# WoojuLee24/OA-DG

Measured on AMD Instinct MI355X. Metric: images/sec training, Faster R-CNN R50-FPN + OA-DG, 1024x2048, higher is better.
Workload: dtype bf16

## Files before the change

oa-dg_amd/csrc/conv_mfma.hip:

```cpp
#include <algorithm>
#include <vector>
#include "common.h"
#include <type_traits>
#include <stdlib.h>
#include "oadg_hip.h"

namespace {

constexpr int BM = 128, BN = 128, BK = 64;

struct ConvArgs {
    const unsigned short* x;
    const unsigned short* w;
    const float* bias;
    const unsigned short* res;
    unsigned short* y;
    const unsigned short* zeros;
    const unsigned short* mask;
    const unsigned char* bits_in;
    unsigned char* bits_out;
    float* colsum;
    int N, H, W, C, K, R, S, Ho, Wo, stride, pad, dil, relu;
    long M;
    int scatter, OH, OW, osh, osw, oph, opw;
    int res_up, lh, lw;
};

__device__ __forceinline__ long out_row(const ConvArgs& a, long m) {
    if (!a.scatter) return m;
    if (a.M <= 0x7fffffffL) {
        const unsigned t = (unsigned)m / (unsigned)a.Wo, wo = (unsigned)m - t * (unsigned)a.Wo;
        const unsigned n = t / (unsigned)a.Ho, ho = t - n * (unsigned)a.Ho;
        return ((long)n * a.OH + (long)ho * a.osh + a.oph) * a.OW + (long)wo * a.osw + a.opw;
    }
    const long t = m / a.Wo;
    const int wo = (int)(m - t * a.Wo);
    const long n = t / a.Ho;
    const int ho = (int)(t - n * a.Ho);
    return (n * a.OH + (long)ho * a.osh + a.oph) * a.OW + (long)wo * a.osw + a.opw;
}

#define OADG_UNIFORM_BRANCH() asm volatile("" ::: "memory")
template <bool POST>
__device__ __forceinline__ bf16x8 finish_piece(const ConvArgs& a, bf16x8 v, const bf16x8 rv, const bf16x8 mv,
                                               float* csum, unsigned mbits = 0xffu, size_t off = 0) {
    if (POST) {
        float f[8];
#pragma unroll
        for (int e = 0; e < 8; ++e) f[e] = bf16_to_f32((unsigned short)v[e]);
        if (a.res) {
            OADG_UNIFORM_BRANCH();
#pragma unroll
            for (int e = 0; e < 8; ++e) f[e] += bf16_to_f32((unsigned short)rv[e]);
            if (a.relu) {
                OADG_UNIFORM_BRANCH();
#pragma unroll
                for (int e = 0; e < 8; ++e) f[e] = fmaxf(f[e], 0.f);
            }
        }
        if (a.mask) {
            OADG_UNIFORM_BRANCH();
#pragma unroll
            for (int e = 0; e < 8; ++e)
                if (!(bf16_to_f32((unsigned short)mv[e]) > 0.f)) f[e] = 0.f;
        }
        if (a.bits_in) {
            OADG_UNIFORM_BRANCH();
#pragma unroll
            for (int e = 0; e < 8; ++e)
                if (!((mbits >> e) & 1u)) f[e] = 0.f;
        }
#pragma unroll
        for (int e = 0; e < 8; ++e) v[e] = (short)f32_to_bf16(f[e]);
    }
    if (a.colsum) {
        OADG_UNIFORM_BRANCH();
#pragma unroll
        for (int e = 0; e < 8; ++e) csum[e] += bf16_to_f32((unsigned short)v[e]);
    }
    if (a.bits_out) {
        OADG_UNIFORM_BRANCH();
        unsigned b = 0;
#pragma unroll
        for (int e = 0; e < 8; ++e) b |= (bf16_to_f32((unsigned short)v[e]) > 0.f ? 1u : 0u) << e;
        a.bits_out[off >> 3] = (unsigned char)b;
    }
    return v;
}

typedef __attribute__((address_space(3))) void* lds_ptr_t;
typedef const __attribute__((address_space(1))) void* gbl_ptr_t;

__device__ __forceinline__ void glds16(const void* g, void* l) {
    __builtin_amdgcn_global_load_lds((gbl_ptr_t)g, (lds_ptr_t)l, 16, 0, 0);
}

template <int TBN, bool POST, int NST, bool PW = false>
__device__ __forceinline__ void conv_igemm_body(const ConvArgs& a, const long bid, unsigned char* smem) {
    constexpr int WN = TBN / 64, WM = 4 / WN, AF = BM / WM / 32, NBP = TBN * 8 / 256;
    constexpr int TSTAGE = (BM + TBN) * BK * 2;
    const int tid = threadIdx.x, lane = tid & 63, wave = tid >> 6;
    const int wm = wave / WN, wn = wave % WN;
    const int n_tiles = a.K / TBN;
    const long m_tiles = (a.M + BM - 1) / BM;
    long mt;
    int nt;
    {
        const long xcd = bid & 7, j = bid >> 3;
        const long per = (m_tiles + 7) >> 3;
        nt = (int)(j % n_tiles);
        mt = PW ? (j / n_tiles) * 8 + xcd : xcd * per + j / n_tiles;
        if (j / n_tiles >= per || mt >= m_tiles) return;
    }
    const long m0 = mt * BM;
    const int k0 = nt * TBN;

    const int cpc = a.C / BK;
    const int nchunks = a.R * a.S * cpc;
    const unsigned short* a_base[4];
    int a_hi0[4], a_wi0[4];
    int seg[4];
    const unsigned short* b_base[4];
#pragma unroll
    for (int i = 0; i < 4; ++i) {
        const int q = i * 256 + tid;
        const int row = q >> 3, slot = q & 7;
        seg[i] = slot ^ ((row >> 1) & 7);
        const long m = m0 + row;
        if (PW) {
            a_base[i] = m < a.M ? a.x + (size_t)m * a.C : nullptr;
            a_hi0[i] = a_wi0[i] = 0;
        } else if (m < a.M) {
            int wo, ho, n;
            if (a.M <= 0x7fffffffL) {
                const unsigned t = (unsigned)m / (unsigned)a.Wo;
                wo = (int)((unsigned)m - t * (unsigned)a.Wo);
                n = (int)(t / (unsigned)a.Ho);
                ho = (int)(t - (unsigned)n * (unsigned)a.Ho);
            } else {
                wo = (int)(m % a.Wo);
                const long t = m / a.Wo;
                ho = (int)(t % a.Ho);
                n = (int)(t / a.Ho);
            }
            a_hi0[i] = ho * a.stride - a.pad;
            a_wi0[i] = wo * a.stride - a.pad;
            a_base[i] = a.x + ((long)n * a.H * a.W + (long)a_hi0[i] * a.W + a_wi0[i]) * a.C + seg[i] * 8;
        } else {
            a_base[i] = nullptr;
            a_hi0[i] = -(1 << 28);
            a_wi0[i] = 0;
        }
        b_base[i] = a.w + (size_t)(k0 + (row < TBN ? row : 0)) * a.R * a.S * a.C + seg[i] * 8;
    }

    int st_r = 0, st_s = 0, st_rs = 0, st_c0 = 0;
    auto stage = [&](int kc, int buf) {
        unsigned char* sa = smem + buf * TSTAGE;
        unsigned char* sb = sa + BM * BK * 2;
        if (PW) {
            const int c0 = kc * BK;
#pragma unroll
            for (int i = 0; i < 4; ++i)
                glds16(a_base[i] ? a_base[i] + c0 + seg[i] * 8 : a.zeros, sa + i * 4096 + wave * 1024);
#pragma unroll
            for (int i = 0; i < NBP; ++i) glds16(b_base[i] + c0, sb + i * 4096 + wave * 1024);
            return;
        }
        const int dr = st_r * a.dil, ds = st_s * a.dil;
        const long aoff = ((long)dr * a.W + ds) * a.C + st_c0;
        const long boff = (long)st_rs * a.C + st_c0;
#pragma unroll
        for (int i = 0; i < 4; ++i) {
            const bool ok = (unsigned)(a_hi0[i] + dr) < (unsigned)a.H && (unsigned)(a_wi0[i] + ds) < (unsigned)a.W;
            glds16(ok ? a_base[i] + aoff : a.zeros, sa + i * 4096 + wave * 1024);
        }
#pragma unroll
        for (int i = 0; i < NBP; ++i) glds16(b_base[i] + boff, sb + i * 4096 + wave * 1024);
// ... 264 lines not shown
        for (int p = 0; p < NS - 1; ++p) stage(range + p * ranges, p);
        request(range, 0);

        auto body = [&](int i, auto set_c) {
            constexpr int set = decltype(set_c)::value;
            const long sub = range + i * ranges;
            OADG_VMCNT((NS - 2) * G + (NS - 1) * (R + S));
            asm volatile("s_barrier" ::: "memory");
            stage(sub + (NS - 1) * ranges, (i + NS - 1) % NS);
            request(sub + ranges, set ^ 1);
            const unsigned char* at = ring + (i % NS) * SUB_BYTES;
            f32x4 acc[RT][CT];
#pragma unroll
            for (int rt = 0; rt < RT; ++rt)
#pragma unroll
                for (int ct = 0; ct < CT; ++ct) acc[rt][ct] = f32x4{0.f, 0.f, 0.f, 0.f};
#pragma unroll
            for (int ks = 0; ks < KS; ++ks) {
                bf16x8 pf[CT];
#pragma unroll
                for (int ct = 0; ct < CT; ++ct)
                    pf[ct] = *reinterpret_cast<const bf16x8*>(at + bbase[ct] + (bsw[ct] ^ (ks * 64)));
#pragma unroll
                for (int rt = 0; rt < RT; ++rt)
#pragma unroll
                    for (int ct = 0; ct < CT; ++ct)
                        acc[rt][ct] = __builtin_amdgcn_mfma_f32_16x16x32_bf16(wf[rt][ks], pf[ct], acc[rt][ct], 0, 0, 0);
            }
#pragma unroll
            for (int rt = 0; rt < RT; ++rt) {
                const f32x4 bv = *reinterpret_cast<const f32x4*>(sbias + rt * 16 + fq * 4);
#pragma unroll
                for (int ct = 0; ct < CT; ++ct) {
                    bf16x4 o;
#pragma unroll
                    for (int r = 0; r < 4; ++r) {
                        float v = acc[rt][ct][r] + bv[r];
                        if (a.relu && !RES) v = fmaxf(v, 0.f);
                        o[r] = (short)f32_to_bf16(v);
                    }
                    *reinterpret_cast<bf16x4*>(stg + (ct * 16 + fr) * STG_STRIDE + (rt * 16 + fq * 4) * 2) = o;
                }
            }
            asm volatile("" ::: "memory");
            if (POST) {
                OADG_VMCNT(S + G + R);
#pragma unroll
                for (int jj = 0; jj < NP; ++jj) {
                    if (RES) asm volatile("" : "+v"(rv[set][jj]));
                    if (BIN) asm volatile("" : "+v"(mb[set][jj]));
                }
            }
#pragma unroll
            for (int jj = 0; jj < NP; ++jj) {
                const int px = ppx + PPP * jj;
                bf16x8 v = *reinterpret_cast<const bf16x8*>(stg + px * STG_STRIDE + psl * 16);
                const size_t off = (size_t)sub * sub_stride + jj * row8 + lane_off;
                v = finish_piece<POST>(a, v, RES ? rv[set][jj] : bf16x8{0, 0, 0, 0, 0, 0, 0, 0}, bf16x8{0, 0, 0, 0, 0, 0, 0, 0},
                                       csum, BIN ? mb[set][jj] : 0xffu, off);
                asm volatile("global_store_dwordx4 %0, %1, off" ::"v"(a.y + off), "v"(v) : "memory");
            }
        };
        OADG_VMCNT(0);
        for (int i = 0; i < n_it; i += 2) {
            body(i, std::integral_constant<int, 0>{});
            if (i + 1 < n_it) body(i + 1, std::integral_constant<int, 1>{});
        }
    }
    if (a.colsum) {
#pragma unroll
        for (int e = 0; e < 8; ++e) {
            float t = csum[e];
#pragma unroll
            for (int sh = LPP; sh < 64; sh <<= 1) t += __shfl_xor(t, sh, 64);
            csum[e] = t;
        }
        if (lane < LPP) {
#pragma unroll
            for (int e = 0; e < 8; ++e) a.colsum[(size_t)range * a.K + kcol + lane * 8 + e] = csum[e];
        }
    }
}

long pw_stream_ranges(long M, int C, int K, int R, int S, int stride, int pad) {
    if (R != 1 || S != 1 || stride != 1 || pad != 0 || (C != 64 && C != 128 && C != 256 && C != 512)) return 0;
    const int kwg = C >= 512 ? 128 : 256;
    if (K % kwg != 0) return 0;
    const int ncol = K / kwg, sp = C >= 256 ? 16 : 32;
    if (ncol > 64 || (64 % ncol) != 0 || M % sp != 0) return 0;
    const long ranges = 512 / ncol;
    return (M / sp) >= 8 * ranges ? ranges : 0;
}

template <int C>
int launch_pw_stream(const ConvArgs& a, hipStream_t st) {
    using Geo = PwGeo<C>;
    const int ncol = a.K / (4 * Geo::KPW);
    const bool res = a.res != nullptr, bin = a.bits_in != nullptr, bout = a.bits_out != nullptr;
#define OADG_PWS(RE, BI, BO)                                                                                       \
    do {                                                                                                           \
        static bool attr = false;                                                                                  \
        if (!attr) {                                                                                               \
            hipError_t e = hipFuncSetAttribute((const void*)conv_pw_stream_kernel<C, RE, BI, BO>,                  \
                                               hipFuncAttributeMaxDynamicSharedMemorySize, Geo::LDS);              \
            if (e != hipSuccess) return (int)e;                                                                    \
            attr = true;                                                                                           \
        }                                                                                                          \
        hipLaunchKernelGGL((conv_pw_stream_kernel<C, RE, BI, BO>), dim3(Geo::GRID), dim3(256), Geo::LDS, st, a, ncol); \
    } while (0)
    if (res && bin && !bout) OADG_PWS(true, true, false);
    else if (res && !bin && bout) OADG_PWS(true, false, true);
    else if (res && !bin && !bout) OADG_PWS(true, false, false);
    else if (!res && bin && !bout) OADG_PWS(false, true, false);
    else if (!res && !bin && bout) OADG_PWS(false, false, true);
    else if (!res && !bin && !bout) OADG_PWS(false, false, false);
    else return OADG_EARG;
#undef OADG_PWS
    return OADG_OK;
}

constexpr int TM = 256, TN = 256;
constexpr int HALF_BYTES = 128 * BK * 2;
constexpr int BUF_BYTES = 4 * HALF_BYTES;

typedef float f32x4v __attribute__((ext_vector_type(4)));

struct TapState {
    int t, r, s, rs, c0;
};

template <bool POST, int NW>
__global__ __launch_bounds__(512) void conv_igemm256_kernel(ConvArgs a) {
    constexpr int TNW = NW * 128;
    extern __shared__ __attribute__((aligned(16))) unsigned char smem[];
    const int tid = threadIdx.x, lane = tid & 63;
    const int wave = __builtin_amdgcn_readfirstlane(tid >> 6);
    const int wr = wave >> 2, wc = wave & 3;
    const int n_tiles = a.K / TNW;
    const long m_tiles = (a.M + TM - 1) / TM;
    const long bid = blockIdx.x;
    long mt;
    int nt;
    {
        const long xcd = bid & 7, j = bid >> 3;
        const long per = (m_tiles + 7) >> 3;
        nt = (int)(j % n_tiles);
        mt = xcd * per + j / n_tiles;
        if (j / n_tiles >= per || mt >= m_tiles) return;
    }
    const long m0 = mt * TM;
    const int k0 = nt * TNW;
    const int nk = a.R * a.S * (a.C / BK);

    const unsigned short* pb[4];
    int hi0[4], wi0[4];
    const unsigned short* wb[4];
#pragma unroll
    for (int h = 0; h < 2; ++h)
#pragma unroll
        for (int i = 0; i < 2; ++i) {
            const int q = i * 512 + tid;
            const int row = q >> 3, lslot = (q & 7) ^ ((row >> 1) & 7);
            const long m = m0 + h * 128 + row;
            if (m < a.M) {
                const unsigned mu = (unsigned)m;
                const unsigned tq = mu / (unsigned)a.Wo;
                const int wo = (int)(mu - tq * (unsigned)a.Wo);
                const int n = (int)(tq / (unsigned)a.Ho);
                const int ho = (int)(tq - (unsigned)n * (unsigned)a.Ho);
                pb[h * 2 + i] = a.x + (size_t)n * a.H * a.W * a.C + lslot * 8;
                hi0[h * 2 + i] = ho * a.stride - a.pad;
                wi0[h * 2 + i] = wo * a.stride - a.pad;
            } else {
                pb[h * 2 + i] = a.x;
                hi0[h * 2 + i] = -(1 << 28);
                wi0[h * 2 + i] = 0;
            }
            wb[h * 2 + i] = a.w + (size_t)(k0 + (h & (NW - 1)) * 128 + row) * a.R * a.S * a.C + lslot * 8;
        }

    auto advance = [&](TapState& st) {
        st.t++;
        st.rs++;
        if (++st.s == a.S) {
            st.s = 0;
            if (++st.r == a.R) { st.r = 0; st.rs = 0; st.c0 += BK; }
        }
    };
    auto stage_pix = [&](int h, const TapState& st, int buf) {
        unsigned char* dst = smem + buf * BUF_BYTES + h * HALF_BYTES + wave * 1024;
        const bool live = st.t < nk;
#pragma unroll
        for (int i = 0; i < 2; ++i) {
            const int hi = hi0[h * 2 + i] + st.r * a.dil, wi = wi0[h * 2 + i] + st.s * a.dil;
            const bool ok = live && (unsigned)hi < (unsigned)a.H && (unsigned)wi < (unsigned)a.W;
            const unsigned short* src = ok ? pb[h * 2 + i] + ((hi * a.W + wi) * a.C + st.c0) : a.zeros;
            glds16(src, dst + i * 8192);
        }
    };
    auto stage_wgt = [&](int h, const TapState& st, int buf) {
        unsigned char* dst = smem + buf * BUF_BYTES + (2 + h) * HALF_BYTES + wave * 1024;
        const bool live = st.t < nk;
#pragma unroll
        for (int i = 0; i < 2; ++i) {
            const unsigned short* src = live ? wb[h * 2 + i] + (st.rs * a.C + st.c0) : a.zeros;
            glds16(src, dst + i * 8192);
        }
    };

    const int fr = lane & 15, fq = lane >> 4;
    int poff[4][2], woff[2][2];
#pragma unroll
    for (int it = 0; it < 4; ++it)
#pragma unroll
        for (int ks = 0; ks < 2; ++ks) {
            const int row = wr * 64 + it * 16 + fr;
            poff[it][ks] = row * 128 + (((ks * 4 + fq) ^ ((row >> 1) & 7)) << 4);
        }
#pragma unroll
    for (int jt = 0; jt < 2; ++jt)
#pragma unroll
        for (int ks = 0; ks < 2; ++ks) {
            const int row = wc * 32 + jt * 16 + fr;
            woff[jt][ks] = row * 128 + (((ks * 4 + fq) ^ ((row >> 1) & 7)) << 4);
        }

    f32x4v acc[NW][2][2][4];
#pragma unroll
    for (int x0 = 0; x0 < NW; ++x0)
#pragma unroll
        for (int x1 = 0; x1 < 2; ++x1)
#pragma unroll
            for (int x2 = 0; x2 < 2; ++x2)
#pragma unroll
                for (int x3 = 0; x3 < 4; ++x3) acc[x0][x1][x2][x3] = f32x4v{0.f, 0.f, 0.f, 0.f};

    bf16x8 pf[4][2], wf[NW][2][2];
    auto read_pix = [&](int h, int buf) {
        const unsigned char* base = smem + buf * BUF_BYTES + h * HALF_BYTES;
#pragma unroll
        for (int it = 0; it < 4; ++it)
#pragma unroll
            for (int ks = 0; ks < 2; ++ks) pf[it][ks] = *reinterpret_cast<const bf16x8*>(base + poff[it][ks]);
    };
    auto read_wgt = [&](int h, int buf) {
        const unsigned char* base = smem + buf * BUF_BYTES + (2 + h) * HALF_BYTES;
#pragma unroll
        for (int jt = 0; jt < 2; ++jt)
#pragma unroll
            for (int ks = 0; ks < 2; ++ks) wf[h][jt][ks] = *reinterpret_cast<const bf16x8*>(base + woff[jt][ks]);
    };
#define OADG_MFMA32(W_FIRST, PH_)                                                                            \
    do {                                                                                                     \
        asm volatile("s_waitcnt lgkmcnt(0)" ::: "memory");                                                   \
        asm volatile("s_barrier" ::: "memory");                                                              \
        __builtin_amdgcn_sched_barrier(0);                                                                   \
        __builtin_amdgcn_s_setprio(1);                                                                       \
        _Pragma("unroll") for (int hh = 0; hh < NW; ++hh)                                                    \
            _Pragma("unroll") for (int ks = 0; ks < 2; ++ks)                                                 \
                _Pragma("unroll") for (int jt = 0; jt < 2; ++jt)                                             \
                    _Pragma("unroll") for (int it = 0; it < 4; ++it)                                         \
                        acc[(hh ^ W_FIRST) & (NW - 1)][jt][PH_][it] = __builtin_amdgcn_mfma_f32_16x16x32_bf16(   \
                            wf[(hh ^ W_FIRST) & (NW - 1)][jt][ks], pf[it][ks],                               \
                            acc[(hh ^ W_FIRST) & (NW - 1)][jt][PH_][it], 0, 0, 0);                           \
        __builtin_amdgcn_s_setprio(0);                                                                       \
        __builtin_amdgcn_sched_barrier(0);                                                                   \
        asm volatile("s_barrier" ::: "memory");                                                              \
    } while (0)

    TapState s1{0, 0, 0, 0, 0};
    stage_pix(0, s1, 0);
    stage_wgt(0, s1, 0);
    if (NW == 2) stage_wgt(1, s1, 0);
    stage_pix(1, s1, 0);
    advance(s1);
    stage_pix(0, s1, 1);
    stage_wgt(0, s1, 1);
    TapState s2 = s1;
    advance(s2);
    asm volatile("s_waitcnt vmcnt(4)" ::: "memory");
    asm volatile("s_barrier" ::: "memory");
    if (wr == 1) asm volatile("s_barrier" ::: "memory");

    for (int t = 0; t < nk; ++t) {
        const int buf = t & 1;
        read_wgt(0, buf);
        if (NW == 2) read_wgt(1, buf);
        read_pix(0, buf);
        if (NW == 2) stage_wgt(1, s1, buf ^ 1);
        stage_pix(1, s1, buf ^ 1);
        OADG_MFMA32(0, 0);
        read_pix(1, buf);
        stage_pix(0, s2, buf);
        stage_wgt(0, s2, buf);
        asm volatile("s_waitcnt vmcnt(4)" ::: "memory");
        OADG_MFMA32(1, 1);
        s1 = s2;
        advance(s2);
    }
#undef OADG_MFMA32
    if (wr == 0) asm volatile("s_barrier" ::: "memory");
    asm volatile("s_waitcnt vmcnt(0)" ::: "memory");
    asm volatile("s_barrier" ::: "memory");

    {
        const int cq = lane >> 4;
#pragma unroll
        for (int wh = 0; wh < NW; ++wh)
#pragma unroll
            for (int jt = 0; jt < 2; ++jt) {
                const int ch = wh * 128 + wc * 32 + jt * 16 + 4 * cq;
                float bv[4] = {0.f, 0.f, 0.f, 0.f};
                if (a.bias) {
#pragma unroll
                    for (int e = 0; e < 4; ++e) bv[e] = a.bias[k0 + ch + e];
                }
#pragma unroll
                for (int ph = 0; ph < 2; ++ph)
#pragma unroll
                    for (int it = 0; it < 4; ++it) {
                        const int p = ph * 128 + wr * 64 + it * 16 + fr;
                        unsigned short o[4];
#pragma unroll
                        for (int e = 0; e < 4; ++e) {
                            float v = acc[wh][jt][ph][it][e] + bv[e];
                            if (a.relu && !a.res) v = fmaxf(v, 0.f);
                            o[e] = f32_to_bf16(v);
                        }
                        uint2 pk;
                        pk.x = (unsigned)o[0] | ((unsigned)o[1] << 16);
                        pk.y = (unsigned)o[2] | ((unsigned)o[3] << 16);
                        *reinterpret_cast<uint2*>(smem + p * (TNW * 2) + ((((ch >> 3) ^ (p & 15))) << 4) + ((ch >> 2) & 1) * 8) = pk;
                    }
            }
    }
    constexpr int NPIECE = (TM * TNW / 8) / 512, SL = TNW / 8;
    bf16x8 rv[POST ? NPIECE : 1], mv[POST ? NPIECE : 1];
    unsigned mb[POST ? NPIECE : 1];
    if (POST) {
#pragma unroll
        for (int it = 0; it < NPIECE; ++it) {
            const int q = it * 512 + tid;
            const long m = m0 + q / SL;
            const size_t off = (size_t)m * a.K + k0 + (q % SL) * 8;
            rv[it] = (a.res && m < a.M) ? *reinterpret_cast<const bf16x8*>(a.res + off) : bf16x8{0, 0, 0, 0, 0, 0, 0, 0};
            mv[it] = (a.mask && m < a.M) ? *reinterpret_cast<const bf16x8*>(a.mask + off) : bf16x8{0, 0, 0, 0, 0, 0, 0, 0};
            mb[it] = (a.bits_in && m < a.M) ? a.bits_in[off >> 3] : 0xffu;
        }
    } else {
        rv[0] = mv[0] = bf16x8{0, 0, 0, 0, 0, 0, 0, 0};
        mb[0] = 0xffu;
    }
    __syncthreads();
    float csum[8] = {0.f, 0.f, 0.f, 0.f, 0.f, 0.f, 0.f, 0.f};
#pragma unroll
    for (int it = 0; it < NPIECE; ++it) {
        const int q = it * 512 + tid;
        const int p = q / SL, sg = q % SL;
        const long m = m0 + p;
        if (m >= a.M) continue;
        bf16x8 v = *reinterpret_cast<const bf16x8*>(smem + p * (TNW * 2) + ((sg ^ (p & 15)) << 4));
        const size_t off = (size_t)m * a.K + k0 + sg * 8;
        *reinterpret_cast<bf16x8*>(a.y + off) = finish_piece<POST>(a, v, rv[POST ? it : 0], mv[POST ? it : 0], csum,
                                                                   mb[POST ? it : 0], off);
    }
    if (a.colsum) {
        float* red = reinterpret_cast<float*>(smem + 2 * BUF_BYTES);
#pragma unroll
        for (int e = 0; e < 8; ++e) red[(tid / SL) * TNW + (tid % SL) * 8 + e] = csum[e];
        __syncthreads();
        if (tid < TNW) {
            float t = 0.f;
#pragma unroll
            for (int g = 0; g < 512 / SL; ++g) t += red[g * TNW + tid];
            a.colsum[(size_t)mt * a.K + k0 + tid] = t;
        }
    }
}

}

namespace {
int auto_variant(long M, int H, int W, int C, int K, int nchunks, int R = 0, int S = 0, int stride = 0, int pad = 0) {
    constexpr bool narrow256 = false;
    const int tnw = K % TN == 0 ? TN : 128;
    const long big = ((M + TM - 1) / TM) * (K / tnw);
    const bool ok256 = (K % TN == 0 || (K == 128 && narrow256)) && big >= 256 && (long)H * W * C < (1L << 31) && M < (1L << 31);
    if (ok256 && nchunks >= 12) return 2;
    if (pw_stream_ranges(M, C, K, R, S, stride, pad) > 0) return 4;
    if (ok256 && nchunks >= 8) return 2;
    const long blocks128 = ((M + BM - 1) / BM) * ((K + 127) / 128);
    if (K % 128 == 0 && blocks128 <= 512 && nchunks >= 32) return 1;
    return 3;
}

static inline bool mask_bits_unused(const void* bits_in, const void* bits_out) { return bits_in != nullptr || bits_out != nullptr; }

int conv_launch(const void* x, const void* w, const float* bias, const void* residual, void* y, const void* zeros16,
                int N, int H, int W, int C, int K, int R, int S, int stride, int pad, int dil, int relu, int variant,
                void* stream, const void* mask = nullptr, float* colsum_part = nullptr, const int* sc = nullptr,
                const void* bits_in = nullptr, void* bits_out = nullptr) {
    if (!x || !w || !y || !zeros16) return OADG_EARG;
    if (N < 1 || H < 1 || W < 1 || R < 1 || S < 1 || stride < 1 || dil < 1 || pad < 0) return OADG_EARG;
    if (C % BK != 0 || K % 64 != 0) return OADG_EARG;
    if (variant < 0 || variant > 4 || (variant == 2 && K % 128 != 0)) return OADG_EARG;
    ConvArgs a;
    a.x = (const unsigned short*)x; a.w = (const unsigned short*)w; a.bias = bias;
    a.res = (const unsigned short*)residual; a.y = (unsigned short*)y; a.zeros = (const unsigned short*)zeros16;
    a.mask = (const unsigned short*)mask; a.colsum = colsum_part;
    a.bits_in = (const unsigned char*)bits_in; a.bits_out = (unsigned char*)bits_out;
    if ((bits_in || bits_out) && K % 8 != 0) return OADG_EARG;
    a.N = N; a.H = H; a.W = W; a.C = C; a.K = K; a.R = R; a.S = S; a.stride = stride; a.pad = pad; a.dil = dil;
    a.relu = relu & 1;
    a.Ho = (H + 2 * pad - dil * (R - 1) - 1) / stride + 1;
    a.Wo = (W + 2 * pad - dil * (S - 1) - 1) / stride + 1;
    a.scatter = 0; a.OH = a.Ho; a.OW = a.Wo; a.osh = a.osw = 1; a.oph = a.opw = 0;
    a.res_up = 0; a.lh = a.lw = 0;
    if (relu & 2) {
        auto lg = [](int v) { int l = 0; while ((1 << l) < v) ++l; return (1 << l) == v ? l : -1; };
        a.lh = lg(H); a.lw = lg(W);
        if (!residual || (H & 1) || (W & 1) || H < 2 || W < 2 || (long)N * H * W >= (1L << 31) || R != 1 || S != 1 || stride != 1 ||
            pad != 0 || sc || mask || mask_bits_unused(bits_in, bits_out))
            return OADG_EARG;
        a.res_up = (a.lh >= 1 && a.lw >= 1) ? 1 : 2;
        a.relu = relu & 1;
        if (variant == 0) variant = 4;
        if (variant != 4) return OADG_EARG;
    }
    if (sc) {
        if (stride != 1 || sc[0] < 1 || sc[1] < 1 || sc[4] < 1 || sc[5] < 1 || sc[6] < 0 || sc[7] < 0) return OADG_EARG;
        if ((long)(sc[0] - 1) * sc[4] + sc[6] >= sc[2] || (long)(sc[1] - 1) * sc[5] + sc[7] >= sc[3]) return OADG_EARG;
        a.Ho = sc[0]; a.Wo = sc[1];
        a.scatter = 1; a.OH = sc[2]; a.OW = sc[3]; a.osh = sc[4]; a.osw = sc[5]; a.oph = sc[6]; a.opw = sc[7];
        if (variant == 0 || variant == 2) variant = 3;
    }
    if (a.Ho < 1 || a.Wo < 1) return OADG_EARG;
    a.M = (long)N * a.Ho * a.Wo;
    const bool post = residual != nullptr || mask != nullptr || bits_in != nullptr;
    if (variant == 0) {
        variant = auto_variant(a.M, H, W, C, K, R * S * (C / BK), R, S, stride, pad);
        if (variant == 4 && (sc || mask || (bits_in && bits_out))) variant = 3;
    }
    if (variant == 2 && ((long)H * W * C >= (1L << 31) || a.M >= (1L << 31))) variant = 1;
    if (variant == 4) {
        if (sc || mask || (bits_in && bits_out) || pw_stream_ranges(a.M, C, K, R, S, stride, pad) == 0) return OADG_EARG;
        int rc = OADG_EARG;
        if (C == 64) rc = launch_pw_stream<64>(a, (hipStream_t)stream);
        else if (C == 128) rc = launch_pw_stream<128>(a, (hipStream_t)stream);
        else if (C == 256) rc = launch_pw_stream<256>(a, (hipStream_t)stream);
        else if (C == 512) rc = launch_pw_stream<512>(a, (hipStream_t)stream);
        if (rc != OADG_OK) return rc;
        OADG_LAUNCH_CHECK();
        return OADG_OK;
    }
    if (variant == 2) {
        static bool attr_set = false;
        if (!attr_set) {
            const void* fns[4] = {(const void*)conv_igemm256_kernel<false, 2>, (const void*)conv_igemm256_kernel<true, 2>,
                                  (const void*)conv_igemm256_kernel<false, 1>, (const void*)conv_igemm256_kernel<true, 1>};
            for (const void* f : fns) {
                hipError_t e = hipFuncSetAttribute(f, hipFuncAttributeMaxDynamicSharedMemorySize, 2 * BUF_BYTES + 16384);
                if (e != hipSuccess) return (int)e;
            }
            attr_set = true;
        }
        const int nw = K % TN == 0 ? 2 : 1;
        const long m_tiles = (a.M + TM - 1) / TM;
        const long blocks = ((m_tiles + 7) / 8) * 8 * (K / (nw * 128));
        if (blocks > 0x7fffffffL) return OADG_EARG;
#define OADG_L256(PO, NW_) \
    hipLaunchKernelGGL((conv_igemm256_kernel<PO, NW_>), dim3((unsigned)blocks), dim3(512), 2 * BUF_BYTES + 16384, (hipStream_t)stream, a)
        if (nw == 2) { if (post) OADG_L256(true, 2); else OADG_L256(false, 2); }
        else { if (post) OADG_L256(true, 1); else OADG_L256(false, 1); }
#undef OADG_L256
    } else {
        const long m_tiles = (a.M + BM - 1) / BM;
        constexpr long tbn64_max = 256;
        const int tbn = (K % BN == 0 && m_tiles * (K / BN) > tbn64_max) ? BN : 64;
        const long blocks = ((m_tiles + 7) / 8) * 8 * (K / tbn);
        if (blocks > 0x7fffffffL) return OADG_EARG;
        const bool one = variant == 3;
        const unsigned lds2 = 2 * (BM + tbn) * BK * 2, lds1 = (BM + tbn) * BK * 2 + 8192;
        hipStream_t st = (hipStream_t)stream;
#define OADG_L128(TB, PO, NS, LDS) \
    hipLaunchKernelGGL((conv_igemm_kernel<TB, PO, NS>), dim3((unsigned)blocks), dim3(256), LDS, st, a)
#define OADG_L128PW(TB, PO, LDS) \
    hipLaunchKernelGGL((conv_igemm_kernel<TB, PO, 1, true>), dim3((unsigned)blocks), dim3(256), LDS, st, a)
        const bool pw = one && R == 1 && S == 1 && stride == 1 && pad == 0 && !a.scatter;
        if (pw) {
            if (tbn == BN) { if (post) OADG_L128PW(128, true, lds1); else OADG_L128PW(128, false, lds1); }
            else { if (post) OADG_L128PW(64, true, lds1); else OADG_L128PW(64, false, lds1); }
        } else if (tbn == BN) {
            if (one) { if (post) OADG_L128(128, true, 1, lds1); else OADG_L128(128, false, 1, lds1); }
            else { if (post) OADG_L128(128, true, 2, lds2); else OADG_L128(128, false, 2, lds2); }
        } else {
            if (one) { if (post) OADG_L128(64, true, 1, lds1); else OADG_L128(64, false, 1, lds1); }
            else { if (post) OADG_L128(64, true, 2, lds2); else OADG_L128(64, false, 2, lds2); }
        }
#undef OADG_L128
#undef OADG_L128PW
    }
    OADG_LAUNCH_CHECK();
    return OADG_OK;
}
}

extern "C" int oadg_conv2d_nhwc_bf16(const void* x, const void* w, const float* bias, const void* residual,
                                     void* y, const void* zeros16, int N, int H, int W, int C, int K, int R,
                                     int S, int stride, int pad, int dil, int relu, void* stream) {
    return conv_launch(x, w, bias, residual, y, zeros16, N, H, W, C, K, R, S, stride, pad, dil, relu, 0, stream);
}

extern "C" int oadg_conv2d_auto_variant(int N, int H, int W, int C, int K, int R, int S, int stride, int pad, int dil) {
    if (N < 1 || H < 1 || W < 1 || R < 1 || S < 1 || stride < 1 || dil < 1 || pad < 0) return 0;
    if (C % BK != 0 || K % 64 != 0) return 0;
    const int Ho = (H + 2 * pad - dil * (R - 1) - 1) / stride + 1, Wo = (W + 2 * pad - dil * (S - 1) - 1) / stride + 1;
    if (Ho < 1 || Wo < 1) return 0;
    return auto_variant((long)N * Ho * Wo, H, W, C, K, R * S * (C / BK), R, S, stride, pad);
}

extern "C" int oadg_conv2d_nhwc_bf16_ex(const void* x, const void* w, const float* bias, const void* residual,
                                        void* y, const void* zeros16, int N, int H, int W, int C, int K, int R, int S,
                                        int stride, int pad, int dil, int relu, int variant, const void* mask,
                                        float* colsum_part, const void* mask_bits, void* relu_bits_out, void* stream) {
    return conv_launch(x, w, bias, residual, y, zeros16, N, H, W, C, K, R, S, stride, pad, dil, relu, variant, stream,
                       mask, colsum_part, nullptr, mask_bits, relu_bits_out);
}

extern "C" int oadg_conv2d_nhwc_bf16_scatter(const void* x, const void* w, const float* bias, const void* residual,
                                             void* y, const void* zeros16, int N, int H, int W, int C, int K, int R,
                                             int S, int pad, int dil, int relu, int out_h, int out_w, int OH, int OW,
                                             int osh, int osw, int oph, int opw, const void* mask,
                                             float* colsum_part, const void* mask_bits, void* stream) {
    const int sc[8] = {out_h, out_w, OH, OW, osh, osw, oph, opw};
    return conv_launch(x, w, bias, residual, y, zeros16, N, H, W, C, K, R, S, 1, pad, dil, relu, 3, stream, mask,
                       colsum_part, sc, mask_bits, nullptr);
}

extern "C" int oadg_conv2d_dgrad_s2_nhwc_bf16(const void* dy, const void* wt, const void* residual, void* dx,
                                              const void* zeros16, int N, int Ho, int Wo, int K, int C, int R, int H, int W,
                                              const void* mask, float* colsum_part, const void* mask_bits, void* stream) {
    if (!dy || !wt || !dx || !zeros16 || N < 1 || Ho < 1 || Wo < 1 || H < 1 || W < 1 || (R != 3 && R != 1)) return OADG_EARG;
    if (K % BK != 0 || C % 64 != 0 || (mask_bits && C % 8 != 0)) return OADG_EARG;
    static const int cls_tab[4][5] = {{0, 0, 1, 1, 0}, {0, 1, 1, 2, 1}, {1, 0, 2, 1, 3}, {1, 1, 2, 2, 5}};
    S2Args g;
    ConvArgs& a = g.base;
    a.x = (const unsigned short*)dy; a.w = nullptr; a.bias = nullptr; a.res = (const unsigned short*)residual;
    a.y = (unsigned short*)dx; a.zeros = (const unsigned short*)zeros16; a.mask = (const unsigned short*)mask;
    a.bits_in = (const unsigned char*)mask_bits; a.bits_out = nullptr; a.colsum = nullptr;
    a.N = N; a.H = Ho; a.W = Wo; a.C = K; a.K = C; a.R = 1; a.S = 1; a.stride = 1; a.pad = 0; a.dil = 1; a.relu = 0;
    a.Ho = a.Wo = 1; a.M = 0;
    a.scatter = 1; a.OH = H; a.OW = W; a.osh = 2; a.osw = 2; a.oph = a.opw = 0;
    a.res_up = 0; a.lh = a.lw = 0;
    const int tbn = (C % BN == 0) ? BN : 64;
    g.n_cls = 0;
    long blocks = 0, rows = 0;
    bool equal = true;
    long first_blocks = -1;
    for (int k = 0; k < (R == 3 ? 4 : 1); ++k) {
        const int ph = cls_tab[k][0], pw = cls_tab[k][1];
        const int ha = (H - ph + 1) / 2, wa = (W - pw + 1) / 2;
        if (ha < 1 || wa < 1) continue;
        if ((long)(ha - 1) * 2 + ph >= H || (long)(wa - 1) * 2 + pw >= W) return OADG_EARG;
        S2Class& c = g.cls[g.n_cls++];
        c.w = (const unsigned short*)wt + (size_t)cls_tab[k][4] * C * K;
        c.R = cls_tab[k][2]; c.S = cls_tab[k][3]; c.Ho = ha; c.Wo = wa; c.oph = ph; c.opw = pw;
        c.M = (long)N * ha * wa;
        const long m_tiles = (c.M + BM - 1) / BM;
        c.colsum = colsum_part ? colsum_part + (size_t)rows * C : nullptr;
        rows += m_tiles;
        const long b = ((m_tiles + 7) / 8) * 8 * (C / tbn);
        if (first_blocks < 0) first_blocks = b;
        equal = equal && b == first_blocks;
        if (blocks + b > 0x7fffffffL) return OADG_EARG;
        c.block0 = (int)blocks;
        blocks += b;
    }
    if (g.n_cls == 0) return OADG_OK;
    for (int k = g.n_cls; k < 4; ++k) g.cls[k] = g.cls[0];
    g.interleave = (g.n_cls == 4 && equal) ? 1 : 0;
    const bool post = residual != nullptr || mask != nullptr || mask_bits != nullptr;
    const unsigned lds1 = (BM + tbn) * BK * 2 + 8192;
    hipStream_t st = (hipStream_t)stream;
#define OADG_LS2(TB, PO) hipLaunchKernelGGL((conv_igemm_s2_kernel<TB, PO>), dim3((unsigned)blocks), dim3(256), lds1, st, g)
    if (tbn == BN) { if (post) OADG_LS2(128, true); else OADG_LS2(128, false); }
    else { if (post) OADG_LS2(64, true); else OADG_LS2(64, false); }
#undef OADG_LS2
    OADG_LAUNCH_CHECK();
    return OADG_OK;
}

extern "C" long oadg_conv2d_pixel_tiles(int N, int H, int W, int C, int K, int R, int S, int stride, int pad, int dil,
                                        int variant) {
    if (variant == 0) variant = oadg_conv2d_auto_variant(N, H, W, C, K, R, S, stride, pad, dil);
    if (variant == 0) return 0;
    const int Ho = (H + 2 * pad - dil * (R - 1) - 1) / stride + 1, Wo = (W + 2 * pad - dil * (S - 1) - 1) / stride + 1;
    const long M = (long)N * Ho * Wo;
    if (variant == 4) return pw_stream_ranges(M, C, K, R, S, stride, pad);
    return variant == 2 ? (M + TM - 1) / TM : (M + BM - 1) / BM;
}

extern "C" int oadg_conv2d_nhwc_bf16_variant(const void* x, const void* w, const float* bias, const void* residual,
                                             void* y, const void* zeros16, int N, int H, int W, int C, int K, int R,
                                             int S, int stride, int pad, int dil, int relu, int variant,
                                             void* stream) {
    return conv_launch(x, w, bias, residual, y, zeros16, N, H, W, C, K, R, S, stride, pad, dil, relu, variant, stream);
}

namespace {

struct WgradArgs {
    const unsigned short* x;
    const unsigned short* dy;
    float* part;
    const unsigned short* zeros;
    int N, H, W, C, K, R, S, Ho, Wo, stride, pad, dil, splits, chunks_per_split;
    int strip_rows;
    long P;
};
// ... 1148 lines not shown
```

Before: 144.4.

## Add row-segment staging path for 3x3 stride-1 convs in 256-tile igemm

Adds a specialized path in the 256-row implicit-GEMM conv kernel for 3x3, stride-1, pad-1 convolutions. It stages whole output-row segments plus a one-pixel halo into LDS once per kernel row and reuses them across the three horizontal taps by shifting fragment addresses. This replaces reloading pixels from global memory for every tap. It uses buffer loads with out-of-bounds offsets to zero-fill padding and is enabled by default when shape conditions hold, with an environment variable to disable it. The tradeoff is more complex LDS addressing and a narrower set of shapes where it applies.

New measurement: 146.2, median of 6. No clear change (+1.2%).

```diff
diff --git a/oa-dg_amd/csrc/conv_mfma.hip b/oa-dg_amd/csrc/conv_mfma.hip
--- a/oa-dg_amd/csrc/conv_mfma.hip
+++ b/oa-dg_amd/csrc/conv_mfma.hip
@@ -24,6 +24,7 @@
     long M;
     int scatter, OH, OW, osh, osw, oph, opw;
     int res_up, lh, lw;
+    int rows;
 };
 
 __device__ __forceinline__ long out_row(const ConvArgs& a, long m) {
@@ -594,78 +595,7 @@
     const int k0 = nt * TNW;
     const int nk = a.R * a.S * (a.C / BK);
 
-    const unsigned short* pb[4];
-    int hi0[4], wi0[4];
-    const unsigned short* wb[4];
-#pragma unroll
-    for (int h = 0; h < 2; ++h)
-#pragma unroll
-        for (int i = 0; i < 2; ++i) {
-            const int q = i * 512 + tid;
-            const int row = q >> 3, lslot = (q & 7) ^ ((row >> 1) & 7);
-            const long m = m0 + h * 128 + row;
-            if (m < a.M) {
-                const unsigned mu = (unsigned)m;
-                const unsigned tq = mu / (unsigned)a.Wo;
-                const int wo = (int)(mu - tq * (unsigned)a.Wo);
-                const int n = (int)(tq / (unsigned)a.Ho);
-                const int ho = (int)(tq - (unsigned)n * (unsigned)a.Ho);
-                pb[h * 2 + i] = a.x + (size_t)n * a.H * a.W * a.C + lslot * 8;
-                hi0[h * 2 + i] = ho * a.stride - a.pad;
-                wi0[h * 2 + i] = wo * a.stride - a.pad;
-            } else {
-                pb[h * 2 + i] = a.x;
-                hi0[h * 2 + i] = -(1 << 28);
-                wi0[h * 2 + i] = 0;
-            }
-            wb[h * 2 + i] = a.w + (size_t)(k0 + (h & (NW - 1)) * 128 + row) * a.R * a.S * a.C + lslot * 8;
-        }
-
-    auto advance = [&](TapState& st) {
-        st.t++;
-        st.rs++;
-        if (++st.s == a.S) {
-            st.s = 0;
-            if (++st.r == a.R) { st.r = 0; st.rs = 0; st.c0 += BK; }
-        }
-    };
-    auto stage_pix = [&](int h, const TapState& st, int buf) {
-        unsigned char* dst = smem + buf * BUF_BYTES + h * HALF_BYTES + wave * 1024;
-        const bool live = st.t < nk;
-#pragma unroll
-        for (int i = 0; i < 2; ++i) {
-            const int hi = hi0[h * 2 + i] + st.r * a.dil, wi = wi0[h * 2 + i] + st.s * a.dil;
-            const bool ok = live && (unsigned)hi < (unsigned)a.H && (unsigned)wi < (unsigned)a.W;
-            const unsigned short* src = ok ? pb[h * 2 + i] + ((hi * a.W + wi) * a.C + st.c0) : a.zeros;
-            glds16(src, dst + i * 8192);
-        }
-    };
-    auto stage_wgt = [&](int h, const TapState& st, int buf) {
-        unsigned char* dst = smem + buf * BUF_BYTES + (2 + h) * HALF_BYTES + wave * 1024;
-        const bool live = st.t < nk;
-#pragma unroll
-        for (int i = 0; i < 2; ++i) {
-            const unsigned short* src = live ? wb[h * 2 + i] + (st.rs * a.C + st.c0) : a.zeros;
-            glds16(src, dst + i * 8192);
-        }
-    };
-
     const int fr = lane & 15, fq = lane >> 4;
-    int poff[4][2], woff[2][2];
-#pragma unroll
-    for (int it = 0; it < 4; ++it)
-#pragma unroll
-        for (int ks = 0; ks < 2; ++ks) {
-            const int row = wr * 64 + it * 16 + fr;
-            poff[it][ks] = row * 128 + (((ks * 4 + fq) ^ ((row >> 1) & 7)) << 4);
-        }
-#pragma unroll
-    for (int jt = 0; jt < 2; ++jt)
-#pragma unroll
-        for (int ks = 0; ks < 2; ++ks) {
-            const int row = wc * 32 + jt * 16 + fr;
-            woff[jt][ks] = row * 128 + (((ks * 4 + fq) ^ ((row >> 1) & 7)) << 4);
-        }
 
     f32x4v acc[NW][2][2][4];
 #pragma unroll
@@ -678,20 +608,6 @@
                 for (int x3 = 0; x3 < 4; ++x3) acc[x0][x1][x2][x3] = f32x4v{0.f, 0.f, 0.f, 0.f};
 
     bf16x8 pf[4][2], wf[NW][2][2];
-    auto read_pix = [&](int h, int buf) {
-        const unsigned char* base = smem + buf * BUF_BYTES + h * HALF_BYTES;
-#pragma unroll
-        for (int it = 0; it < 4; ++it)
-#pragma unroll
-            for (int ks = 0; ks < 2; ++ks) pf[it][ks] = *reinterpret_cast<const bf16x8*>(base + poff[it][ks]);
-    };
-    auto read_wgt = [&](int h, int buf) {
-        const unsigned char* base = smem + buf * BUF_BYTES + (2 + h) * HALF_BYTES;
-#pragma unroll
-        for (int jt = 0; jt < 2; ++jt)
-#pragma unroll
-            for (int ks = 0; ks < 2; ++ks) wf[h][jt][ks] = *reinterpret_cast<const bf16x8*>(base + woff[jt][ks]);
-    };
 #define OADG_MFMA32(W_FIRST, PH_)                                                                            \
     do {                                                                                                     \
         asm volatile("s_waitcnt lgkmcnt(0)" ::: "memory");                                                   \
@@ -710,35 +626,261 @@
         asm volatile("s_barrier" ::: "memory");                                                              \
     } while (0)
 
-    TapState s1{0, 0, 0, 0, 0};
-    stage_pix(0, s1, 0);
-    stage_wgt(0, s1, 0);
-    if (NW == 2) stage_wgt(1, s1, 0);
-    stage_pix(1, s1, 0);
-    advance(s1);
-    stage_pix(0, s1, 1);
-    stage_wgt(0, s1, 1);
-    TapState s2 = s1;
-    advance(s2);
-    asm volatile("s_waitcnt vmcnt(4)" ::: "memory");
-    asm volatile("s_barrier" ::: "memory");
-    if (wr == 1) asm volatile("s_barrier" ::: "memory");
-
-    for (int t = 0; t < nk; ++t) {
-        const int buf = t & 1;
-        read_wgt(0, buf);
-        if (NW == 2) read_wgt(1, buf);
-        read_pix(0, buf);
-        if (NW == 2) stage_wgt(1, s1, buf ^ 1);
-        stage_pix(1, s1, buf ^ 1);
-        OADG_MFMA32(0, 0);
-        read_pix(1, buf);
-        stage_pix(0, s2, buf);
-        stage_wgt(0, s2, buf);
+    if (!a.rows) {
+        const unsigned short* pb[4];
+        int hi0[4], wi0[4];
+        const unsigned short* wb[4];
+#pragma unroll
+        for (int h = 0; h < 2; ++h)
+#pragma unroll
+            for (int i = 0; i < 2; ++i) {
+                const int q = i * 512 + tid;
+                const int row = q >> 3, lslot = (q & 7) ^ ((row >> 1) & 7);
+                const long m = m0 + h * 128 + row;
+                if (m < a.M) {
+                    const unsigned mu = (unsigned)m;
+                    const unsigned tq = mu / (unsigned)a.Wo;
+                    const int wo = (int)(mu - tq * (unsigned)a.Wo);
+                    const int n = (int)(tq / (unsigned)a.Ho);
+                    const int ho = (int)(tq - (unsigned)n * (unsigned)a.Ho);
+                    pb[h * 2 + i] = a.x + (size_t)n * a.H * a.W * a.C + lslot * 8;
+                    hi0[h * 2 + i] = ho * a.stride - a.pad;
+                    wi0[h * 2 + i] = wo * a.stride - a.pad;
+                } else {
+                    pb[h * 2 + i] = a.x;
+                    hi0[h * 2 + i] = -(1 << 28);
+                    wi0[h * 2 + i] = 0;
+                }
+                wb[h * 2 + i] = a.w + (size_t)(k0 + (h & (NW - 1)) * 128 + row) * a.R * a.S * a.C + lslot * 8;
+            }
+
+        auto advance = [&](TapState& st) {
+            st.t++;
+            st.rs++;
+            if (++st.s == a.S) {
+                st.s = 0;
+                if (++st.r == a.R) { st.r = 0; st.rs = 0; st.c0 += BK; }
+            }
+        };
+        auto stage_pix = [&](int h, const TapState& st, int buf) {
+            unsigned char* dst = smem + buf * BUF_BYTES + h * HALF_BYTES + wave * 1024;
+            const bool live = st.t < nk;
+#pragma unroll
+            for (int i = 0; i < 2; ++i) {
+                const int hi = hi0[h * 2 + i] + st.r * a.dil, wi = wi0[h * 2 + i] + st.s * a.dil;
+                const bool ok = live && (unsigned)hi < (unsigned)a.H && (unsigned)wi < (unsigned)a.W;
+                const unsigned short* src = ok ? pb[h * 2 + i] + ((hi * a.W + wi) * a.C + st.c0) : a.zeros;
+                glds16(src, dst + i * 8192);
+            }
+        };
+        auto stage_wgt = [&](int h, const TapState& st, int buf) {
+            unsigned char* dst = smem + buf * BUF_BYTES + (2 + h) * HALF_BYTES + wave * 1024;
+            const bool live = st.t < nk;
+#pragma unroll
+            for (int i = 0; i < 2; ++i) {
+                const unsigned short* src = live ? wb[h * 2 + i] + (st.rs * a.C + st.c0) : a.zeros;
+                glds16(src, dst + i * 8192);
+            }
+        };
+        int poff[4][2], woff[2][2];
+#pragma unroll
+        for (int it = 0; it < 4; ++it)
+#pragma unroll
+            for (int ks = 0; ks < 2; ++ks) {
+                const int row = wr * 64 + it * 16 + fr;
+                poff[it][ks] = row * 128 + (((ks * 4 + fq) ^ ((row >> 1) & 7)) << 4);
+            }
+#pragma unroll
+        for (int jt = 0; jt < 2; ++jt)
+#pragma unroll
+            for (int ks = 0; ks < 2; ++ks) {
+                const int row = wc * 32 + jt * 16 + fr;
+                woff[jt][ks] = row * 128 + (((ks * 4 + fq) ^ ((row >> 1) & 7)) << 4);
+            }
+        auto read_pix = [&](int h, int buf) {
+            const unsigned char* base = smem + buf * BUF_BYTES + h * HALF_BYTES;
+#pragma unroll
+            for (int it = 0; it < 4; ++it)
+#pragma unroll
+                for (int ks = 0; ks < 2; ++ks) pf[it][ks] = *reinterpret_cast<const bf16x8*>(base + poff[it][ks]);
+        };
+        auto read_wgt = [&](int h, int buf) {
+            const unsigned char* base = smem + buf * BUF_BYTES + (2 + h) * HALF_BYTES;
+#pragma unroll
+            for (int jt = 0; jt < 2; ++jt)
+#pragma unroll
+                for (int ks = 0; ks < 2; ++ks) wf[h][jt][ks] = *reinterpret_cast<const bf16x8*>(base + woff[jt][ks]);
+        };
+
+        TapState s1{0, 0, 0, 0, 0};
+        stage_pix(0, s1, 0);
+        stage_wgt(0, s1, 0);
+        if (NW == 2) stage_wgt(1, s1, 0);
+        stage_pix(1, s1, 0);
+        advance(s1);
+        stage_pix(0, s1, 1);
+        stage_wgt(0, s1, 1);
+        TapState s2 = s1;
+        advance(s2);
         asm volatile("s_waitcnt vmcnt(4)" ::: "memory");
-        OADG_MFMA32(1, 1);
-        s1 = s2;
-        advance(s2);
+        asm volatile("s_barrier" ::: "memory");
+        if (wr == 1) asm volatile("s_barrier" ::: "memory");
+
+        for (int t = 0; t < nk; ++t) {
+            const int buf = t & 1;
+            read_wgt(0, buf);
+            if (NW == 2) read_wgt(1, buf);
+            read_pix(0, buf);
+            if (NW == 2) stage_wgt(1, s1, buf ^ 1);
+            stage_pix(1, s1, buf ^ 1);
+            OADG_MFMA32(0, 0);
+            read_pix(1, buf);
+            stage_pix(0, s2, buf);
+            stage_wgt(0, s2, buf);
+            asm volatile("s_waitcnt vmcnt(4)" ::: "memory");
+            OADG_MFMA32(1, 1);
+            s1 = s2;
+            advance(s2);
+        }
+    } else {
+        constexpr int ROWS_SEG_BYTES = 5 * 8192, ROWS_SEG0 = 4 * HALF_BYTES;
+        constexpr unsigned OOB = 0xFFFFF000u;
+        const int segL = a.Wo < TM ? a.Wo : TM;
+        const int segE = segL + 2;
+        const int segN = (TM / segL) * segE;
+        const int G = nk / 3;
+        const __amdgpu_buffer_rsrc_t xr = __builtin_amdgcn_make_buffer_rsrc(
+            (void*)a.x, 0, (unsigned)((size_t)a.N * a.H * a.W * a.C * 2), 0x00020000);
+        const __amdgpu_buffer_rsrc_t wrs = __builtin_amdgcn_make_buffer_rsrc(
+            (void*)a.w, 0, (unsigned)((size_t)a.K * 9 * a.C * 2), 0x00020000);
+        unsigned so[5];
+        unsigned vbits = 0;
+#pragma unroll
+        for (int i = 0; i < 5; ++i) {
+            const int c = i * 512 + tid;
+            const int e = c >> 3, lslot = (c & 7) ^ ((e >> 1) & 7);
+            so[i] = 0;
+            if (e < segN) {
+                const int jr = e / segE, col = e - jr * segE;
+                const long ms = m0 + (long)jr * segL;
+                if (ms < a.M) {
+                    const unsigned mu = (unsigned)ms;
+                    const unsigned tq = mu / (unsigned)a.Wo;
+                    const int wo0 = (int)(mu - tq * (unsigned)a.Wo);
+                    const int n = (int)(tq / (unsigned)a.Ho);
+                    const int ho = (int)(tq - (unsigned)n * (unsigned)a.Ho);
+                    const int wi = wo0 + col - 1;
+                    if ((unsigned)wi < (unsigned)a.W) {
+                        so[i] = ((((unsigned)n * a.H + (unsigned)(ho - 1)) * a.W + (unsigned)wi) * a.C + lslot * 8) * 2u;
+#pragma unroll
+                        for (int r = 0; r < 3; ++r)
+                            if ((unsigned)(ho - 1 + r) < (unsigned)a.H) vbits |= 1u << (3 * i + r);
+                    }
+                }
+            }
+        }
+        const int last_waves = (segN - 256 + 7) >> 3;
+        const int wrow = tid >> 3;
+        const unsigned wo00 = ((unsigned)(k0 + wrow) * 9 * a.C + (((tid & 7) ^ ((wrow >> 1) & 7)) * 8)) * 2u;
+        const unsigned wstep64 = 64u * 9 * a.C * 2u;
+        struct Group { int g, r, c0; };
+        auto next_group = [&](Group& q) {
+            q.g++;
+            if (++q.r == 3) { q.r = 0; q.c0 += BK; }
+        };
+        auto stage_seg = [&](int i, const Group& q) {
+            unsigned o = (unsigned)__builtin_amdgcn_readfirstlane((q.r * a.W * a.C + q.c0) * 2);
+            asm volatile("" : "+s"(o));
+            const unsigned bit = q.g < G ? 1u << (3 * i + q.r) : 0u;
+            const unsigned vo = (vbits & bit) ? so[i] + o : OOB;
+            __builtin_amdgcn_raw_ptr_buffer_load_lds(
+                xr, (lds_ptr_t)(smem + ROWS_SEG0 + (q.g & 1) * ROWS_SEG_BYTES + i * 8192 + wave * 1024), 16, (int)vo, 0, 0, 0);
+        };
+        auto stage_w = [&](int h, const Group& q, int s, int buf) {
+            unsigned char* dst = smem + buf * (2 * HALF_BYTES) + h * HALF_BYTES + wave * 1024;
+            unsigned o = (unsigned)__builtin_amdgcn_readfirstlane(q.g < G ? ((q.r * 3 + s) * a.C + q.c0) * 2 : 0);
+            asm volatile("" : "+s"(o));
+#pragma unroll
+            for (int i = 0; i < 2; ++i)
+                __builtin_amdgcn_raw_ptr_buffer_load_lds(wrs, (lds_ptr_t)(dst + i * 8192), 16,
+                                                         (int)(wo00 + (o + (h * 2 + i) * wstep64)), 0, 0, 0);
+        };
+        const int jb0 = ((wr * 64 + fr) + 2 * ((wr * 64 + fr) / segL)) * 128;
+        const int jb1 = (128 + 2 * (128 / segL)) * 128;
+        int fa;
+        auto frag_addr = [&](int ph, int s, int g) {
+            int j128 = jb0 + (ph * jb1 + s * 128);
+            asm volatile("" : "+v"(j128));
+            fa = (j128 | (((j128 >> 4) & 0x70) ^ (tid & 0x30))) + (g & 1) * ROWS_SEG_BYTES;
+            asm volatile("" : "+v"(fa));
+        };
+        auto read_seg = [&]() {
+            const unsigned char* b0 = smem + ROWS_SEG0 + fa;
+            const unsigned char* b1 = smem + ROWS_SEG0 + (fa ^ 64);
+#pragma unroll
+            for (int it = 0; it < 4; ++it) {
+                pf[it][0] = *reinterpret_cast<const bf16x8*>(b0 + it * 2048);
+                pf[it][1] = *reinterpret_cast<const bf16x8*>(b1 + it * 2048);
+            }
+        };
+        const int w0 = (wc * 32 + fr) * 128 + ((fq ^ (((wc * 32 + fr) >> 1) & 7)) << 4);
+        auto read_w = [&](int h, int buf) {
+            const unsigned char* b0 = smem + buf * (2 * HALF_BYTES) + h * HALF_BYTES + w0;
+            const unsigned char* b1 = smem + buf * (2 * HALF_BYTES) + h * HALF_BYTES + (w0 ^ 64);
+#pragma unroll
+            for (int jt = 0; jt < 2; ++jt) {
+                wf[h][jt][0] = *reinterpret_cast<const bf16x8*>(b0 + jt * 2048);
+                wf[h][jt][1] = *reinterpret_cast<const bf16x8*>(b1 + jt * 2048);
+            }
+        };
+
+        Group cur{0, 0, 0};
+#pragma unroll
+        for (int i = 0; i < 5; ++i) stage_seg(i, cur);
+        stage_w(0, cur, 0, 0);
+        if (NW == 2) stage_w(1, cur, 0, 0);
+        stage_w(0, cur, 1, 1);
+        Group nxt = cur;
+        next_group(nxt);
+        asm volatile("s_waitcnt vmcnt(2)" ::: "memory");
+        asm volatile("s_barrier" ::: "memory");
+        if (wr == 1) asm volatile("s_barrier" ::: "memory");
+        frag_addr(0, 0, 0);
+
+        for (int g = 0; g < G; ++g) {
+#pragma unroll
+            for (int u = 0; u < 3; ++u) {
+                const int buf = (g + u) & 1;
+                read_seg();
+                read_w(0, buf);
+                if (NW == 2) read_w(1, buf);
+                frag_addr(1, u, g);
+                if (NW == 2) {
+                    if (u < 2) stage_w(1, cur, u + 1, buf ^ 1); else stage_w(1, nxt, 0, buf ^ 1);
+                }
+                if (u == 1) stage_seg(2, nxt);
+                if (u == 2 && wave < last_waves) stage_seg(4, nxt);
+                OADG_MFMA32(0, 0);
+                read_seg();
+                frag_addr(0, u == 2 ? 0 : u + 1, u == 2 ? g + 1 : g);
+                if (u == 0) {
+                    stage_w(0, cur, 2, buf);
+                    stage_seg(0, nxt);
+                    stage_seg(1, nxt);
+                    asm volatile("s_waitcnt vmcnt(4)" ::: "memory");
+                } else if (u == 1) {
+                    stage_w(0, nxt, 0, buf);
+                    stage_seg(3, nxt);
+                    asm volatile("s_waitcnt vmcnt(3)" ::: "memory");
+                } else {
+                    stage_w(0, nxt, 1, buf);
+                    asm volatile("s_waitcnt vmcnt(2)" ::: "memory");
+                }
+                OADG_MFMA32(1, 1);
+            }
+            cur = nxt;
+            next_group(nxt);
+        }
     }
 #undef OADG_MFMA32
     if (wr == 0) asm volatile("s_barrier" ::: "memory");
@@ -858,6 +1000,7 @@
     a.Wo = (W + 2 * pad - dil * (S - 1) - 1) / stride + 1;
     a.scatter = 0; a.OH = a.Ho; a.OW = a.Wo; a.osh = a.osw = 1; a.oph = a.opw = 0;
     a.res_up = 0; a.lh = a.lw = 0;
+    a.rows = 0;
     if (relu & 2) {
         auto lg = [](int v) { int l = 0; while ((1 << l) < v) ++l; return (1 << l) == v ? l : -1; };
         a.lh = lg(H); a.lw = lg(W);
@@ -907,6 +1050,10 @@
             attr_set = true;
         }
         const int nw = K % TN == 0 ? 2 : 1;
+        const char* rows_env = getenv("OADG_CONV256_ROWS");
+        a.rows = R == 3 && S == 3 && stride == 1 && dil == 1 && pad == 1 && a.Wo % 64 == 0 &&
+                 (a.Wo % TM == 0 || TM % a.Wo == 0) && (size_t)N * H * W * C * 2 < 0xFFFFF000ul &&
+                 (size_t)K * 9 * C * 2 < 0xFFFFF000ul && !(rows_env && rows_env[0] == '0');
         const long m_tiles = (a.M + TM - 1) / TM;
         const long blocks = ((m_tiles + 7) / 8) * 8 * (K / (nw * 128));
         if (blocks > 0x7fffffffL) return OADG_EARG;
```
